# pymc-devs/pymc

Hardware: AMD Instinct MI355X
Metric: effective samples/sec (and leapfrog steps/sec), 10k-param hierarchical logistic regression, one NUTS chain per GPU (higher is better)
Workload: dtype f64

## Files before the change

pymc_amd/csrc/engine.hip:

```cpp
#include <hip/hip_runtime.h>

#include <algorithm>
#include <atomic>
#include <chrono>
#include <cmath>
#include <cstdio>
#include <cstdlib>
#include <cstring>
#include <mutex>
#include <thread>
#include <utility>
#include <ctime>
#include <string>
#include <vector>

#include "kernels.h"
#include "small_kernel.h"
#include "mixture_kernel.h"
#include "loglik_kernel.h"
#include "predictive_kernel.h"
#include "summary_kernel.h"
#include "nuts_mi355.h"
#include "pcg64_stream.h"
#include "advi.h"
// ... 17 lines not shown
static int env_int(const char* name, int dflt) {
  std::lock_guard<std::mutex> lk(g_opt_mu);
  for (const auto& kv : g_opts) if (kv.first == name) return kv.second;
  return dflt;
}
extern "C" int nuts_set_option(const char* name, int32_t value) {
  if (!name || std::strncmp(name, "NUTS_", 5) != 0) { g_err = "option names start with NUTS_"; return NUTS_E_ARG; }
  std::lock_guard<std::mutex> lk(g_opt_mu);
  for (auto& kv : g_opts) if (kv.first == name) { kv.second = value; return NUTS_OK; }
  g_opts.emplace_back(name, value);
  return NUTS_OK;
}
extern "C" void nuts_clear_options(void) {
  std::lock_guard<std::mutex> lk(g_opt_mu);
  g_opts.clear();
}

template <typename T>
static T* dev_alloc(size_t count) {
  void* p = nullptr;
  const size_t bytes = std::max<size_t>(count, 1) * sizeof(T);
  if (hipMalloc(&p, bytes) != hipSuccess) return nullptr;
  if (env_int("NUTS_POISON_ALLOC", 0)) { hipMemset(p, 0xFF, bytes); hipDeviceSynchronize(); }
  return static_cast<T*>(p);
}
template <typename T>
static T* dev_upload(const T* src, size_t count) {
  T* p = dev_alloc<T>(count);
  if (p && count) hipMemcpy(p, src, count * sizeof(T), hipMemcpyHostToDevice);
  return p;
}

enum { EP_PLAIN = 0, EP_PAIRED = 1, EP_REPLAY = 2 };
struct EdgePlan {
  int ring = 64;
  int side = 0, n = 0;
  unsigned head = 0;
  int cap = 0, used = 0;
  int64_t ring_full = 0;
  void reset() { side = 0; n = 0; cap = 0; used = 0; }
  template <class F>
  void begin(int d, int dir, int last, F dir_of) {
    cap = 0; used = 0;
    for (int e = d + 1; e <= last; ++e)
      if (dir_of(e) == -dir) { cap = std::min(1 << std::min(e, 30), ring); break; }
  }
  int leaf(int dir, int* slot, int* k) {
    if (n > 0 && side == dir) { *slot = (int)(head % (unsigned)ring); *k = used++; ++head; --n; return EP_REPLAY; }
    if (cap > 0 && n < cap) { side = -dir; *k = n; *slot = (int)((head + (unsigned)n) % (unsigned)ring); ++n; return EP_PAIRED; }
    if (cap > 0 && n >= ring) ++ring_full;
    *slot = -1; *k = -1;
    return EP_PLAIN;
  }
};
extern "C" int64_t nuts_edge_pair_plan(const int32_t* dirs, int32_t n_dirs, int32_t n_doublings, int32_t spec, int32_t max_depth,
                                       int32_t ring, int32_t* out, int64_t out_cap) {
  if (!dirs || !out || n_doublings < 0 || n_doublings > n_dirs || n_doublings > 20 || ring < 1) { g_err = "nuts_edge_pair_plan: bad argument"; return -1; }
  EdgePlan ep;
  ep.ring = ring;
  int64_t n = 0;
  const int last = std::min(std::min(spec, max_depth - 1), n_dirs - 1);
  for (int d = 0; d < n_doublings; ++d) {
    ep.begin(d, dirs[d], last, [&](int e) { return (int)dirs[e]; });
    for (int j = 0; j < (1 << d); ++j, ++n) {
      int slot, k;
      const int kind = ep.leaf(dirs[d], &slot, &k);
// ... 17 lines not shown
  double* g_dev = nullptr;
  double* lp_dev = nullptr;
  double* host_pin = nullptr;
  std::vector<nuts_data_ref> data_refs;
  int64_t data_epoch = 0;
  double* set_pin = nullptr; int64_t set_pin_len = 0; hipEvent_t set_ev = nullptr;
  int rows_grid = 0, mvn_grid = 0, ept = 1;
  bool has_prog = false;
  int rows_rpl = 2, rows_alternate = 1, rows_flip = 0, rows_occ = 4;
  int vector_one_xcd = 0;
  int ga_struct_ok = 0;
  int ga_par = 0;
  int64_t dom_units = 0;
  int explicit_pre = 0;
  int64_t alg_bytes = 0;
  bool profile = false;
  std::vector<hipEvent_t> ev;
  std::vector<int32_t> ev_units;
  int run_open = 0;
  int64_t runs_seen = 0;
  size_t ev_used = 0;
  int64_t dom_launches = 0;
  int sample_every = 1;
  hipStream_t own_stream = nullptr;
  struct nuts_group* group = nullptr;
  bool g_active = false;
  int gslot = 0;
  int n_chains = 0;
  int64_t pool_extra = 0;
  int64_t orphan_elems = 0, factor_elems = 0;
  double rows_pack_s = 0.0;
  int64_t rows_xt_len = 0, rows_y_len = 0;
  int ep_ok = 0, ep_par = 0;
  double *ep_ring = nullptr, *ep_part = nullptr, *ep_bpart = nullptr, *ep_def_loc = nullptr;
  int64_t ep_ring_bytes = 0, ep_shadows = 0, ep_replays = 0;
  int64_t ep_dropped = 0;
  int64_t ep_ring_full = 0;
  int ep_turns = 0;
  struct EpLaunch {
    int kind = EP_PLAIN, slot = 0, sj = 0, sfold = 0, first = 0;
    EvalIO sio{}; ArenaDev sA{};
  } ep_launch;
  std::vector<LinDev> lins_host;
  std::vector<nuts_factor> fac_host;
  double *ll_q = nullptr, *ll_stage = nullptr, *ll_par = nullptr, *ll_sc = nullptr, *ll_lfact = nullptr;
  int32_t* ll_dead = nullptr;
  int64_t ll_stage_n = 0, ll_par_n = 0;
  int n_waic = 0;

  template <typename T>
  T* keep(T* p) {
    owned.push_back((void*)p);
    return p;
  }
};

extern "C" int nuts_device_count(void) {
  int n = 0;
  if (hipGetDeviceCount(&n) != hipSuccess) return 0;
  return n;
}
extern "C" int nuts_set_device(int device) {
  HIPCHK(hipSetDevice(device));
  return NUTS_OK;
}
extern "C" const char* nuts_last_error(void) { return g_err.c_str(); }
// ... 351 lines not shown
#undef GLM_LAUNCH
    if (prof) { hipEventRecord(m->ev[m->ev_used + 1], m->stream); m->ev_used += 2; m->dom_units += 1; }
    m->dom_launches++;
    hipLaunchKernelGGL(k_glm_reduce, dim3((md.glm.Ppad + 3 + GLM_RED_COLS - 1) / GLM_RED_COLS), dim3(GLM_RED_CHUNKS * GLM_RED_COLS), 0, m->stream, md, A, io, j);
    if (!md.has_mvn) return;
    prof = false; m->dom_launches--;
  }
  if (md.has_logit && md.lg.ga) {
    const int rev = m->rows_alternate ? (m->rows_flip ^= 1) : 0;
    const int par = (m->ga_par ^= 1);
    const dim3 grid(m->rows_grid + (fold ? 1 : 0) + md.lg.ga_naux), block(WAVE * md.lg.ga_w);
    GaArgs ga{md, A, io, j, rev, fold ? (GA_FOLD_CTL | GA_FOLD_SRC) : 0, par, d, max_depth, Emax, st, io, j - 1, d, 0, 0};
    if (fold && job) {
      ga.fold = GA_FOLD_CTL | (job->src_prev ? GA_FOLD_SRC : 0);
      ga.cio = job->io; ga.cj = job->j; ga.cd = job->d; ga.cseq = job->seq;
    }
    const nuts_model::EpLaunch ep = m->ep_launch;
    m->ep_launch.kind = EP_PLAIN;
    if (ep.kind == EP_PAIRED) {
      GaMultiArgs<2, true> ma;
      GaLeafArgs& L = ma.c[0];
      L.A = A; L.io = io; L.cio = ga.cio; L.Emax = Emax; L.st = st;
      L.ga_part = md.lg.ga_part; L.ga_bpart = md.lg.ga_bpart; L.ga_ticket = md.lg.ga_ticket; L.def_loc = md.def_loc;
      L.j = j; L.fold = ga.fold; L.par = par; L.d = d; L.max_depth = max_depth; L.cj = ga.cj; L.cd = ga.cd; L.cseq = ga.cseq;
      L.slot = 0; L.pad = 0;
      GaLeafArgs& S = ma.c[1];
      S.A = ep.sA; S.io = ep.sio; S.cio = ep.sio; S.Emax = Emax; S.st = nullptr;
      S.ga_part = m->ep_part; S.ga_bpart = m->ep_bpart; S.ga_ticket = md.lg.ga_ticket + md.lg.ga_nblk; S.def_loc = m->ep_def_loc;
      S.j = ep.sj; S.fold = ep.sfold; S.par = (m->ep_par ^= 1); S.d = 0; S.max_depth = 1; S.cj = 0; S.cd = 0; S.cseq = 0;
      S.slot = GAM_MAXC - 1; S.pad = ep.first ? GAM_SH_FIRST : 0;
      ma.rev = rev; ma.pad = 0;
      ma.ring = m->ep_ring + (size_t)ep.slot * md.lg.G * GA_RING_DOUBLES(8);
      const dim3 pgrid(GAM_MAXC + md.lg.G);
      if (md.lg.ga_dx == 7) hipLaunchKernelGGL((k_rows_ga_multi<2, 3, 7, true>), pgrid, block, 0, m->stream, md, ma);
      else hipLaunchKernelGGL((k_rows_ga_multi<2, 3, 8, true>), pgrid, block, 0, m->stream, md, ma);
      m->ep_shadows++;
    } else if (ep.kind == EP_REPLAY) {
      const dim3 rgrid(m->rows_grid + (fold ? 1 : 0));
      hipLaunchKernelGGL((k_rows_ga_replay<8>), rgrid, block, 0, m->stream, ga,
                         (const double*)(m->ep_ring + (size_t)ep.slot * md.lg.G * GA_RING_DOUBLES(8)));
      m->ep_replays++;
    } else
    if (m->group && m->g_active && io.mode == MODE_TREE && m->group->kind >= 2) {
      GaLeafArgs L;
      L.A = A; L.io = io; L.cio = ga.cio; L.Emax = Emax; L.st = st;
      L.ga_part = md.lg.ga_part; L.ga_bpart = md.lg.ga_bpart; L.ga_ticket = md.lg.ga_ticket; L.def_loc = md.def_loc;
      L.j = j; L.fold = ga.fold; L.par = par; L.d = d; L.max_depth = max_depth; L.cj = ga.cj; L.cd = ga.cd; L.cseq = ga.cseq;
      L.slot = m->gslot; L.pad = 0;
      group_deposit(m, L);
    } else
    if (md.lg.ga_gpw) {
      switch (md.lg.D) {
        case 8: if (md.lg.ga_dx == 7) hipLaunchKernelGGL((k_rows_gb<8, 7>), grid, block, 0, m->stream, ga);
                else hipLaunchKernelGGL((k_rows_gb<8>), grid, block, 0, m->stream, ga); break;
        case 4: hipLaunchKernelGGL((k_rows_gb<4>), grid, block, 0, m->stream, ga); break;
        case 2: hipLaunchKernelGGL((k_rows_gb<2>), grid, block, 0, m->stream, ga); break;
        case 1: hipLaunchKernelGGL((k_rows_gb<1>), grid, block, 0, m->stream, ga); break;
        case 3: hipLaunchKernelGGL((k_rows_gb<3>), grid, block, 0, m->stream, ga); break;
        case 5: hipLaunchKernelGGL((k_rows_gb<5>), grid, block, 0, m->stream, ga); break;
        case 6: hipLaunchKernelGGL((k_rows_gb<6>), grid, block, 0, m->stream, ga); break;
        default: hipLaunchKernelGGL((k_rows_gb<7>), grid, block, 0, m->stream, ga); break;
      }
    } else {
      switch (md.lg.D) {
        case 8: if (md.lg.ga_pack) hipLaunchKernelGGL((k_rows_ga<8, 2, 7, 1>), grid, block, 0, m->stream, ga);
                else if (md.lg.ga_dx == 7) hipLaunchKernelGGL((k_rows_ga<8, 2, 7>), grid, block, 0, m->stream, ga);
                else hipLaunchKernelGGL((k_rows_ga<8, 2>), grid, block, 0, m->stream, ga); break;
        case 4: hipLaunchKernelGGL((k_rows_ga<4, 2>), grid, block, 0, m->stream, ga); break;
// ... 657 lines not shown
        int t = -1;
        for (int u = 0; u < md.n_derived; ++u) if (md.derived_f[u] == fi) t = u;
        if (t < 0) { g_err = "linear predictor: coefficients must be a variable or a NUTS_D_DERIVED factor"; return false; }
        const int64_t sz = cs.fac[fi].size;
        if (last >= sz) { g_err = "linear predictor: coefficients beyond the end of their derived vector"; return false; }
        C.transform = -1; C.lower = 0.0; C.upper = 0.0;
        cbase = md.derived_off[t]; dst_base = const_cast<double*>(md.pool) + md.derived_off[t] + sz;
      }
      for (int p = 0; p < L.P; ++p) {
        const int64_t e = (int64_t)L.off[k] + (int64_t)p * L.stride[k];
        coef[(size_t)k * L.P + p] = (int32_t)(cbase + e);
        if (C.n_use > 0) srcs.push_back(Src{(int64_t)reinterpret_cast<intptr_t>(dst_base + e), LinSrc{l, k, p, 0}, dst_base + e});
      }
    }
    D.coef = m->keep(dev_upload(coef.data(), coef.size()));
    m->alg_bytes += 16 * L.N * (int64_t)L.P;
  }
  std::stable_sort(srcs.begin(), srcs.end(), [](const Src& a, const Src& b) { return a.key < b.key; });
  std::vector<LinTarget> targets;
  std::vector<LinSrc> flat;
  for (size_t i = 0; i < srcs.size(); ++i) {
    if (i == 0 || srcs[i].key != srcs[i - 1].key) targets.push_back(LinTarget{srcs[i].dst, (int32_t)flat.size(), 0});
    targets.back().n_src++;
    flat.push_back(srcs[i].src);
  }
  md.n_lins = s->n_lins; md.n_lin_targets = (int32_t)targets.size();
  md.lins = m->keep(dev_upload(m->lins_host.data(), m->lins_host.size()));
  md.lin_targets = m->keep(dev_upload(targets.data(), targets.size()));
  md.lin_srcs = m->keep(dev_upload(flat.data(), flat.size()));
  return true;
}

static bool build_rows_group(nuts_model* m, const nuts_model_spec* s, const std::vector<int64_t>& gptr, const std::vector<int32_t>& tile0,
                             int64_t maxT, int W, int gpw) {
  RowsDev& lg = m->md.lg;
  const int n = m->md.n, D = lg.D, SPAN = WAVE * m->rows_rpl;
  const int64_t n_tiles = tile0[lg.G];
  lg.ga = 1; lg.ga_w = gpw ? GB_W : W;
  lg.ga_gpw = gpw;
  lg.ga_bsz = gpw ? gpw : (lg.G + 31) / 32;
  lg.ga_flags = env_int("NUTS_GA_FLAGS", 0);
  lg.ga_T_uni = 0; lg.ga_ng_uni = 0;
  {
    bool uni = lg.G > 0;
    for (int g = 1; g < lg.G; ++g) uni = uni && (gptr[g + 1] - gptr[g] == gptr[1] - gptr[0]);
    if (uni && maxT > 0) { lg.ga_T_uni = (int32_t)maxT; lg.ga_ng_uni = gptr[1] - gptr[0]; }
  }
  lg.ga_nblk = (lg.G + lg.ga_bsz - 1) / lg.ga_bsz;
  lg.ga_auxel = n - lg.G * D;
  lg.ga_naux = m->ga_struct_ok == 2 ? (lg.ga_auxel + WAVE * lg.ga_w - 1) / (WAVE * lg.ga_w) : 0;
  lg.ga_nrec = lg.ga_nblk + lg.ga_naux;
  bool ones0 = D == 8 && env_int("NUTS_GA_ONES0", 1) != 0 && lg.N > 0;
  for (int64_t i = 0; ones0 && i < lg.N; ++i) ones0 = s->rows_X[i * D] == 1.0;
  const int DX = ones0 ? D - 1 : D;
  lg.ga_dx = DX;
  const int64_t TS = (int64_t)DX * SPAN, GA_SKEW = env_int("NUTS_GA_SKEW", DX == 7 || DX == 5 ? 1120 : 1056);
  if (GA_SKEW % DX != 0) return refuse("NUTS_GA_SKEW must be a multiple of the stored column count");
  std::vector<int64_t> coff((size_t)lg.G * W, 0);
  int64_t pos = 0, max_ct = 0;
  for (int g = 0; g < lg.G; ++g) {
    const int64_t T = tile0[g + 1] - tile0[g];
    for (int w = 0; w < W; ++w) {
      const int64_t ct = (int64_t)(w + 1) * T / W - (int64_t)w * T / W;
      coff[(size_t)g * W + w] = pos;
      pos += ct * TS + GA_SKEW;
      max_ct = std::max(max_ct, ct);
    }
// ... 62 lines not shown
      }
      exc.push_back(RpExc{0, 0, 0, 0});
      lg.Xp = m->keep(dev_upload(xp.data(), xp.size()));
      lg.ga_pcoff = m->keep(dev_upload(pcoff.data(), pcoff.size()));
      lg.ga_pexc_idx = m->keep(dev_upload(exc_idx.data(), exc_idx.size()));
      lg.ga_pexc = m->keep(dev_upload(exc.data(), exc.size()));
      lg.ga_pack_ebase20 = (uint32_t)plan.elo << 20;
      lg.ga_pack = (lg.Xp && lg.ga_pcoff && lg.ga_pexc_idx && lg.ga_pexc) ? 1 : 0;
      if (!lg.ga_pack) (void)hipGetLastError();
    }
    m->rows_pack_s = std::chrono::duration<double>(std::chrono::steady_clock::now() - t0).count();
  }
  lg.ga_coff = m->keep(dev_upload(coff.data(), coff.size()));
  lg.ga_tile0 = m->keep(dev_upload(tile0.data(), tile0.size()));
  lg.ga_part = m->keep(dev_alloc<double>((size_t)lg.G * PART_STRIDE));
  const size_t bpart_len = gpw ? 2 * (size_t)PART_STRIDE * ((lg.ga_nrec + WAVE - 1) / WAVE * WAVE) : 2 * (size_t)lg.ga_nrec * PART_STRIDE;
  lg.ga_bpart = m->keep(dev_alloc<double>(bpart_len));
  lg.ga_ticket = m->keep(dev_alloc<unsigned>(2 * (size_t)lg.ga_nblk));
  if (lg.ga_part) hipMemset(lg.ga_part, 0, (size_t)lg.G * PART_STRIDE * sizeof(double));
  if (lg.ga_bpart) hipMemset(lg.ga_bpart, 0, bpart_len * sizeof(double));
  if (lg.ga_ticket) hipMemset(lg.ga_ticket, 0, 2 * (size_t)lg.ga_nblk * sizeof(unsigned));
  m->ep_ok = 0;
  if (!gpw && D == 8 && m->rows_rpl == 2 && m->ga_struct_ok == 1 && lg.ga_naux == 0 && env_int("NUTS_EDGE_PAIR", 1) != 0) {
    const size_t ring_len = (size_t)GA_RING_LEAVES * lg.G * GA_RING_DOUBLES(8);
    m->ep_ring = m->keep(dev_alloc<double>(ring_len));
    m->ep_part = m->keep(dev_alloc<double>((size_t)lg.G * PART_STRIDE));
    m->ep_bpart = m->keep(dev_alloc<double>(bpart_len));
    m->ep_def_loc = m->keep(dev_alloc<double>(2 * 4 * (size_t)MAX_DEFERRED));
    if (m->ep_ring && m->ep_part && m->ep_bpart && m->ep_def_loc) {
      hipMemset(m->ep_part, 0, (size_t)lg.G * PART_STRIDE * sizeof(double));
      hipMemset(m->ep_bpart, 0, bpart_len * sizeof(double));
      hipMemset(m->ep_def_loc, 0, 2 * 4 * (size_t)MAX_DEFERRED * sizeof(double));
      m->ep_ok = 1; m->ep_ring_bytes = (int64_t)(ring_len * sizeof(double));
    } else (void)hipGetLastError();
  }
  m->rows_grid = gpw ? lg.ga_nblk : lg.G;
  return true;
}

static bool build_rows_spans(nuts_model* m, const nuts_model_spec* s, int cus) {
  RowsDev& lg = m->md.lg;
  const int D = lg.D, SPAN = WAVE * m->rows_rpl;
  const int32_t* gid = s->rows_gid;
  int wpc = env_int("NUTS_ROWS_WAVES_PER_CU", 0);
  if (wpc <= 0) {
    const int64_t spans = (s->rows_N + (int64_t)WAVE * m->rows_rpl - 1) / ((int64_t)WAVE * m->rows_rpl);
    wpc = spans >= (int64_t)cus * 32 * 4 ? 32 : 16;
  }
  {
    std::vector<double> xt((size_t)D * lg.Npad, 0.0);
    for (int64_t i = 0; i < lg.N; ++i) {
      const int64_t sp = i / SPAN, r = i % SPAN;
      for (int d = 0; d < D; ++d) xt[((size_t)sp * D + d) * SPAN + r] = s->rows_X[i * D + d];
    }
    lg.Xt = m->keep(dev_upload(xt.data(), xt.size()));
  }
  std::vector<int8_t> yy(lg.Npad, 0);
  for (int64_t i = 0; i < lg.N; ++i) yy[i] = s->rows_y[i];
  lg.y = m->keep(dev_upload(yy.data(), yy.size()));
  const int waves_per_block = ROWS_BLOCK / WAVE;
  int64_t want_waves = std::min<int64_t>((int64_t)cus * wpc, lg.n_spans);
  const int nb_main = (int)((want_waves + waves_per_block - 1) / waves_per_block);
  lg.n_waves = nb_main * waves_per_block;
  std::vector<int32_t> span_gid(lg.n_spans), mixed_g0, mixed_seg_base, mixed_seg_gid;
  std::vector<int64_t> mixed_span;
  for (int64_t sp = 0; sp < lg.n_spans; ++sp) {
// ... 86 lines not shown
    if (i > 0 && gid[i] < gid[i - 1]) return refuse("logit rows: group ids must be sorted");
    if (gid[i] < 0 || gid[i] >= lg.G) return refuse("logit rows: group id out of range");
    gptr[gid[i] + 1] = i + 1;
  }
  for (int g = 0; g < lg.G; ++g) gptr[g + 1] = std::max(gptr[g + 1], gptr[g]);
  lg.gptr = m->keep(dev_upload(gptr.data(), gptr.size()));
  const int want = (s->rows_opts & NUTS_ROWS_NO_GROUP_ALIGNED) ? 0 : env_int("NUTS_ROWS_GA", 1);
  std::vector<int32_t> tile0(lg.G + 1, 0);
  int64_t maxT = 0;
  for (int g = 0; g < lg.G; ++g) {
    const int64_t T = (gptr[g + 1] - gptr[g] + SPAN - 1) / SPAN;
    maxT = std::max(maxT, T);
    tile0[g + 1] = tile0[g] + (int32_t)T;
  }
  const int64_t n_tiles = tile0[lg.G];
  int W = std::min(GA_MAXW, (16 * cus) / std::max(lg.G, 1));
  if (env_int("NUTS_ROWS_GA_W", 0) > 0) W = std::max(1, std::min(GA_MAXW, env_int("NUTS_ROWS_GA_W", 0)));
  const double meanT = (double)n_tiles / std::max(lg.G, 1);
  bool use = false;
  if (want >= 2) { use = m->ga_struct_ok && m->ept == 1; W = std::max(1, W); }
  else if (want == 1) use = m->ga_struct_ok && m->ept == 1 && W >= 1 && lg.G >= 2 * cus && meanT >= 4.0 * W && (double)maxT <= 1.5 * meanT + 1.0;
  int gpw = 0;
  if (!use && want == 1 && !(s->rows_opts & NUTS_ROWS_NO_GROUP_BLOCK) && env_int("NUTS_ROWS_GB", 1) && m->ga_struct_ok && m->ept == 1 &&
      lg.G >= 64 && maxT <= 16) {
    gpw = GB_W * (int)((lg.G + GB_W * 512 - 1) / (GB_W * 512));
    gpw = std::min(gpw, GB_MAXGPW);
    if (env_int("NUTS_ROWS_GPW", 0) > 0) gpw = std::max(1, std::min(GB_MAXGPW, env_int("NUTS_ROWS_GPW", 0)));
    const int aux_threads = WAVE * GB_W, auxel = n - lg.G * D;
    const int naux = m->ga_struct_ok == 2 ? (auxel + aux_threads - 1) / aux_threads : 0;
    if ((lg.G + gpw - 1) / gpw + naux > WAVE * SLOT_SUM_MAXR) gpw = 0;
  }
  if (gpw) { use = true; W = 1; }
  const bool group = use && n_tiles * (int64_t)SPAN < ((int64_t)1 << 31) && (gpw || lg.G <= 32 * 8 * GA_MAXCHUNK);
  if (!(group ? build_rows_group(m, s, gptr, tile0, maxT, W, gpw) : build_rows_spans(m, s, cus))) return false;
  m->alg_bytes += lg.N * (8 * (int64_t)D + 1 + 4);
  return true;
}

static bool build_mvn(nuts_model* m, const nuts_model_spec* s) {
  ModelDev& md = m->md;
  if (s->mvn_k <= 0) return true;
  const int n = md.n;
  md.has_mvn = 1;
  m->explicit_pre = 1;
  MvnDev& mv = md.mv;
  mv.k = s->mvn_k; mv.off = s->vars[s->mvn_var].offset;
  mv.mu = m->keep(dev_upload(s->mvn_mu, mv.k));
  mv.prec = m->keep(dev_upload(s->mvn_prec, (size_t)mv.k * mv.k));
  mv.rowq = m->keep(dev_alloc<double>(mv.k));
  mv.gdense = m->keep(dev_alloc<double>(n));
  hipMemset(mv.gdense, 0, n * sizeof(double));
  mv.konst = -0.5 * mv.k * std::log(2.0 * M_PI) - s->mvn_logdet;
  mv.winv = nullptr; mv.winv_t = nullptr; mv.wy = nullptr;
  if (s->mvn_winv) {
    const size_t kk = (size_t)mv.k * mv.k;
    std::vector<double> wt(kk);
    for (int r = 0; r < mv.k; ++r)
      for (int cc = 0; cc < mv.k; ++cc) wt[(size_t)cc * mv.k + r] = s->mvn_winv[(size_t)r * mv.k + cc];
    mv.winv = m->keep(dev_upload(s->mvn_winv, kk));
    mv.winv_t = m->keep(dev_upload(wt.data(), kk));
    mv.wy = m->keep(dev_alloc<double>(3 * (size_t)mv.k));
  }
  m->mvn_grid = mv.k;
  m->alg_bytes += 8 * (int64_t)mv.k * mv.k;
  mv.aligned = 0; mv.al_nwg = 0; mv.al_part = nullptr;
  if (md.lean_ok && !md.has_logit && !mv.winv && mv.off == 0 && mv.k == n && s->n_vars == 1 && s->n_factors == 0 &&
      s->vars[0].transform == NUTS_TR_NONE && md.n_deferred == 0 && md.n_orphans == 0) {
// ... 161 lines not shown
  md.has_glm = 1;
  m->alg_bytes += 8 * gm.N * (int64_t)gm.P;
  return true;
}

static bool model_build(nuts_model* m, const nuts_model_spec* s) {
  ModelDev& md = m->md;
  HIPCHK_FALSE(hipStreamCreateWithFlags(&m->stream, hipStreamNonBlocking));
  m->own_stream = m->stream;
  int n = 0;
  for (int i = 0; i < s->n_vars; ++i) n = std::max(n, s->vars[i].offset + s->vars[i].size);
  md.n = n; md.n_vars = s->n_vars; md.n_factors = s->n_factors; md.n_data = s->n_data;
  md.fdead_mode = 0;
  md.fdead = m->keep(dev_alloc<int32_t>((size_t)std::max(s->n_factors, 1)));
  if (md.fdead) hipMemset(md.fdead, 0, (size_t)std::max(s->n_factors, 1) * sizeof(int32_t));
  CompiledSpec cs;
  if (!compile_spec(m, s, cs)) return false;
  m->fac_host = cs.fac;
  {
    double* pool = m->keep(dev_alloc<double>((size_t)std::max<int64_t>(s->data_pool_len + m->pool_extra, 1)));
    if (pool) {
      hipMemset(pool, 0, (size_t)std::max<int64_t>(s->data_pool_len + m->pool_extra, 1) * sizeof(double));
      if (s->data_pool_len > 0) hipMemcpy(pool, s->data_pool, (size_t)s->data_pool_len * sizeof(double), hipMemcpyHostToDevice);
    }
    md.pool = pool;
    md.pool_len = (int32_t)std::min<int64_t>(s->data_pool_len + m->pool_extra, INT32_MAX);
  }
  m->data_refs.assign(s->data, s->data + s->n_data);
  m->ept = n <= 65536 ? 1 : (n <= 262144 ? 4 : 16);
  md.nblk = (n + VEC_THREADS * m->ept - 1) / (VEC_THREADS * m->ept);
  if (m->orphan_elems > 4 * VEC_THREADS * (int64_t)md.nblk)
    md.nblk = (int)std::min<int64_t>(256, (m->orphan_elems + 4 * VEC_THREADS - 1) / (4 * VEC_THREADS));
  md.tick_j = env_int("NUTS_TICK_J", -1);
  md.ticks = m->keep(dev_alloc<long long>(64));
  hipMemset(md.ticks, 0, 64 * sizeof(long long));
  md.part_stride = PART_STRIDE;
  m->vector_one_xcd = env_int("NUTS_VECTOR_ONE_XCD", 0);
  md.part = m->keep(dev_alloc<double>((size_t)md.nblk * PART_STRIDE));
  hipMemset(md.part, 0, (size_t)md.nblk * PART_STRIDE * sizeof(double));
  m->q_dev = m->keep(dev_alloc<double>(n));
  m->g_dev = m->keep(dev_alloc<double>(n));
  m->lp_dev = m->keep(dev_alloc<double>(2));
  HIPCHK_FALSE(hipHostMalloc((void**)&m->host_pin, (2 * (size_t)n + 2) * sizeof(double), hipHostMallocDefault));
  m->alg_bytes = 0;

  hipDeviceProp_t prop;
  int dev = 0;
  hipGetDevice(&dev);
  hipGetDeviceProperties(&prop, dev);
  const int cus = prop.multiProcessorCount > 0 ? prop.multiProcessorCount : 256;
  if (!build_rows(m, s, cus) || !build_mvn(m, s) || !build_mix(m, s, cs) || !build_glm(m, s, cs, cus) || !build_lins(m, s, cs) ||
      !build_sweep_fast(m, s, cs))
    return false;
  for (void* p : m->owned)
    if (!p) return refuse("device allocation failed");
  HIPCHK_FALSE(hipDeviceSynchronize());
  return true;
}

extern "C" nuts_model* nuts_model_create(const nuts_model_spec* s) {
  if (!s || s->n_vars <= 0) { g_err = "empty model spec"; return nullptr; }
  int ndev = 0;
  if (hipGetDeviceCount(&ndev) != hipSuccess || ndev == 0) {
    g_err = "no HIP device visible: libnuts_mi355 requires an MI355X (gfx950); there is no CPU fallback";
    return nullptr;
  }
  auto* m = new nuts_model();
  if (!model_build(m, s)) { nuts_model_destroy(m); return nullptr; }
// ... 35 lines not shown
    const int64_t off0 = m->data_refs[data_ids[i]].offset;
    int64_t run = lens[i];
    int j = i + 1;
    while (j < count && m->data_refs[data_ids[j]].offset == off0 + run) { run += lens[j]; ++j; }
    if (run > 0)
      HIPCHK(hipMemcpyAsync(const_cast<double*>(m->md.pool) + off0, m->set_pin + at, (size_t)run * sizeof(double), hipMemcpyHostToDevice, m->stream));
    at += run;
    i = j;
  }
  HIPCHK(hipEventRecord(m->set_ev, m->stream));
  m->data_epoch++;
  return NUTS_OK;
}

static void group_remove_model(struct nuts_group* g, nuts_model* m);
extern "C" void nuts_model_destroy(nuts_model* m) {
  if (!m) return;
  if (m->stream) hipStreamSynchronize(m->stream);
  if (m->set_ev) hipEventDestroy(m->set_ev);
  if (m->set_pin) hipHostFree(m->set_pin);
  if (m->group) group_remove_model(m->group, m);
  for (void* p : m->owned) if (p) hipFree(p);
  for (void* p : {(void*)m->ll_q, (void*)m->ll_stage, (void*)m->ll_par, (void*)m->ll_sc, (void*)m->ll_dead, (void*)m->ll_lfact}) if (p) hipFree(p);
  for (auto e : m->ev) hipEventDestroy(e);
  if (m->host_pin) hipHostFree(m->host_pin);
  if (m->own_stream) hipStreamDestroy(m->own_stream);
  delete m;
}

extern "C" int nuts_model_debug_ticks(nuts_model* m, int64_t* out) {
  if (!m || !out) return NUTS_E_ARG;
  HIPCHK(hipStreamSynchronize(m->stream));
  HIPCHK(hipMemcpy(out, m->md.ticks, 64 * sizeof(long long), hipMemcpyDeviceToHost));
  return NUTS_OK;
}

extern "C" int32_t nuts_model_ndim(const nuts_model* m) { return m ? m->md.n : -1; }
extern "C" int nuts_model_get_scalar(const nuts_model* m, const char* name, double* out) {
  if (!m || !name || !out) return NUTS_E_ARG;
  const std::string k(name);
  if (k == "rows_group_aligned") *out = m->md.lg.ga;
  else if (k == "rows_group_block") *out = m->md.lg.ga_gpw;
  else if (k == "rows_packed") *out = m->md.lg.ga ? m->md.lg.ga_pack : 0;
  else if (k == "rows_pack_build_s") *out = m->rows_pack_s;
  else if (k == "edge_pair") *out = m->ep_ok;
  else if (k == "edge_pair_ring_bytes") *out = (double)m->ep_ring_bytes;
  else if (k == "edge_pair_shadows") *out = (double)m->ep_shadows;
  else if (k == "edge_pair_replays") *out = (double)m->ep_replays;
  else if (k == "edge_pair_turns") *out = m->ep_turns;
  else if (k == "edge_pair_dropped") *out = (double)m->ep_dropped;
  else if (k == "edge_pair_ring_full") *out = (double)m->ep_ring_full;
  else if (k == "rows_aux_workgroups") *out = m->md.lg.ga ? m->md.lg.ga_naux : 0;
  else if (k == "mixture_workgroups") *out = m->md.has_mix ? m->md.mix.nwg : 0;
  else if (k == "glm_workgroups") *out = m->md.has_glm ? m->md.glm.nwg : 0;
  else if (k == "glm_row_stride") *out = m->md.has_glm ? m->md.glm.xstride : 0;
  else if (k == "glm_layout_width") *out = m->md.has_glm ? m->md.glm.Ppad : 0;
  else if (k == "mvn_row_aligned") *out = m->md.has_mvn ? m->md.mv.aligned : 0;
  else if (k == "loglik_batch") *out = LL_B;
  else if (k == "loglik_stage_bytes") *out = (double)(m->ll_stage_n * LL_B * (int64_t)sizeof(double));
  else if (k == "rows_waves") *out = m->md.lg.ga ? m->md.lg.ga_w : m->md.lg.n_waves;
  else if (k == "lean") *out = m->md.lean_ok;
  else if (k == "chain_group_kind") {
    const RowsDev& lg = m->md.lg;
    const bool is_mvn = m->md.has_mvn && (m->md.mv.aligned == 4 || m->md.mv.aligned == 8 || m->md.mv.aligned == 16);
    const bool is_rows = m->md.has_logit && !m->md.has_mvn && lg.ga && lg.ga_naux == 0 && lg.D == 8 && m->ga_struct_ok == 1;
    *out = is_mvn ? 1.0 : (is_rows ? (lg.ga_gpw > 0 ? 3.0 : 2.0) : 0.0);
  }
  else if (k == "chain_group_wide_ok") *out = (m->md.has_mvn && m->md.mv.aligned > 0 && m->md.mv.k % 16 == 0) ? 1.0 : 0.0;
  else if (k == "chain_group_wide_rows") *out = 8.0;
  else if (k == "single_workgroup_ok") *out = (m->md.n <= SMALL_MAX_N && m->ept == 1 && !m->md.has_logit && !m->md.has_mvn && !m->md.has_mix && !m->md.has_glm && m->md.n_lins == 0 && m->factor_elems <= SMALL_MAX_ELEMS) ? 1.0 : 0.0;
  else { g_err = "unknown model scalar " + k; return NUTS_E_ARG; }
  return NUTS_OK;
}
extern "C" int64_t nuts_model_algorithmic_bytes(const nuts_model* m) { return m ? m->alg_bytes : 0; }

extern "C" int nuts_model_logp_grad(nuts_model* m, const double* q, double* logp, double* grad) {
  if (!m || !q || !logp) { g_err = "null argument"; return NUTS_E_ARG; }
  const int n = m->md.n;
  std::memcpy(m->host_pin, q, n * sizeof(double));
  HIPCHK(hipMemcpyAsync(m->q_dev, m->host_pin, n * sizeof(double), hipMemcpyHostToDevice, m->stream));
  m->md.fdead_mode = 1;
  model_enqueue_plain(m, m->q_dev, m->g_dev, m->lp_dev);
  m->md.fdead_mode = 0;
  HIPCHK(hipMemcpyAsync(m->host_pin + n, m->g_dev, n * sizeof(double), hipMemcpyDeviceToHost, m->stream));
// ... 2754 lines not shown
```

pymc_amd/csrc/model_dev.h:

```cpp
#pragma once
#include "device_math.h"
#include "nuts_mi355.h"
#include "rows_pack.h"

#define MAX_BTERMS 8
#define MAX_DERIVED 4
#define MAX_FACTOR_BT 6
#define MAX_DEFERRED 256
#define LOGIT_MAXD 8
#define SEG_MAIN_MAX 10

struct VarDev {
  int32_t offset, size, transform, deferred;
  double lower, upper;
  int32_t normal_prior;
  int32_t def_base;
  double np_mu, np_inv_var, np_lognorm;
};

struct Contrib {
  int32_t f;
  int16_t arg, slot;
  int32_t owner;
  int32_t fast;
// ... 173 lines not shown
  int64_t derived_off[MAX_DERIVED];
  const char* prog;
  int32_t po_vars, po_cptr, po_contrib, po_factors, po_fbt, po_btvar, po_data, po_deferred, po_instrs, po_pad;
  long long* ticks;
  int32_t tick_j;
  int32_t fdead_mode;
  int32_t* fdead;
  int32_t n_gsf, n_gs_elems;
  int32_t po_gsf, po_gslot;
  int32_t n_gs_blocks, n_orphans_b;
  double* gs_part;
  int32_t n_swf, sw_bytes, sw_rows, sw_po_leaf, sw_po_instr, sw_po_slot;
  int32_t sw_max_leaves, sw_max_slots, sw_max_instr, sw_blocks;
  const char* sw_blob;
  int32_t gs_lds_rows, gs_lds_bytes;
  double* adj;
  int32_t n_glong, glong_pad;
  const GLong* glong;
  double* adj_red;
  int32_t n_lins, n_lin_targets;
  const LinDev* lins;
  const LinTarget* lin_targets;
  const LinSrc* lin_srcs;
  double* lin_gdense;
};

#ifdef NUTS_KTIMING
__device__ __forceinline__ long long tick_now() {
  unsigned long long t;
  asm volatile("s_waitcnt vmcnt(0) lgkmcnt(0)\n\ts_memtime %0\n\ts_waitcnt lgkmcnt(0)" : "=s"(t) :: "memory");
  return (long long)t;
}
#define TICK(md, cond, slot) do { if (cond) (md).ticks[slot] = tick_now(); } while (0)
#else
#define TICK(md, cond, slot) do { } while (0)
#endif

__device__ __forceinline__ void st_agent(double* p, double v) {
  __hip_atomic_store(reinterpret_cast<unsigned long long*>(p), (unsigned long long)__double_as_longlong(v), __ATOMIC_RELAXED,
                     __HIP_MEMORY_SCOPE_AGENT);
}
__device__ __forceinline__ double ld_agent(const double* p) {
  return __longlong_as_double((long long)__hip_atomic_load(reinterpret_cast<const unsigned long long*>(p), __ATOMIC_RELAXED,
                                                           __HIP_MEMORY_SCOPE_AGENT));
}

template <int BATCH = 8>
__device__ __forceinline__ double sum_strided(const double* base, int stride, int s0, int s1) {
  double acc = 0.0;
  for (int s = s0; s < s1; s += BATCH) {
    double v[BATCH];
#pragma unroll
    for (int u = 0; u < BATCH; ++u) v[u] = base[(int64_t)min(s + u, s1 - 1) * stride];
#pragma unroll
    for (int u = 0; u < BATCH; ++u) acc += (s + u < s1) ? v[u] : 0.0;
  }
  return acc;
}

#define CTL_CHUNKS 8

__device__ __forceinline__ double deferred_finish(double gx_local, double S, double dxdq, double dj) {
  return fma(gx_local + S, dxdq, dj);
}

#define PROG_LDS_MAX 12288

// ... 783 lines not shown
```

pymc_amd/csrc/rows_ga_multi_kernel.h:

```cpp
#pragma once
#include "mvn_multi_kernel.h"

#define GAM_MAXC 8
#define GAM_MAXNC 4

struct GaLeafArgs {
  ArenaDev A;
  EvalIO io, cio;
  double Emax;
  HostStatus* st;
  double* ga_part;
  double* ga_bpart;
  unsigned* ga_ticket;
  double* def_loc;
  int j, fold, par, d, max_depth, cj, cd, cseq;
  int slot, pad;
};

template <int NC, bool SH = false>
struct GaMultiArgs {
  GaLeafArgs c[NC];
  int rev, pad;
};
#define GAM_SH_FIRST 1
template <int NC>
struct GaMultiArgs<NC, true> {
  GaLeafArgs c[NC];
  int rev, pad;
  double* ring;
};

__device__ __forceinline__ LeanSrc gam_src(const RowsDev& R, const GaLeafArgs& L, int par) {
  return LeanSrc{L.ga_bpart + (int64_t)par * R.ga_nrec * PART_STRIDE, PART_STRIDE, R.ga_nrec, L.def_loc + (int64_t)par * 4 * MAX_DEFERRED};
}

template <int DX>
__device__ __forceinline__ void gam_load(const double* base , const int8_t* ybase, int lane,
                                         typename GaTileSel<DX>::type& t) {
  const ga_v2d* p = reinterpret_cast<const ga_v2d*>(base) + lane;
#pragma unroll
  for (int k = 0; k < DX; ++k) t.c[k] = p[k * WAVE];
  t.y = *reinterpret_cast<const uint16_t*>(ybase + 2 * lane);
}

template <int NC, int OCC, int DX, bool SH = false>
__global__ __launch_bounds__(64 * GA_MAXW, OCC) void k_rows_ga_multi(ModelDev md, GaMultiArgs<NC, SH> ma) {
  constexpr int D = 8, RPL = 2, SPAN = WAVE * RPL, PIPE = 2;
  static_assert(!SH || NC == 2, "edge pairing: the chain's leaf and one shadow leaf");
  typedef GaMultiArgs<NC, SH> Args;
  typedef typename GaTileSel<DX>::type Tile;
  const RowsDev& R = md.lg;
  if ((int)blockIdx.x < GAM_MAXC) {
    int ci = -1;
#pragma unroll
    for (int c = 0; c < NC; ++c) ci = (int)blockIdx.x == ma.c[c].slot ? c : ci;
    if (ci < 0) return;
    const GaLeafArgs& L = ma.c[ci];
    if (L.fold & GA_FOLD_CTL) control_lean(md, L.A, L.cio, L.cj, L.cd, L.Emax, L.max_depth, L.st, L.cseq, gam_src(R, L, L.par ^ 1));
    return;
  }
  const int g = (int)blockIdx.x - GAM_MAXC;
  const int rev = ma.rev;
  const int tid = threadIdx.x, lane = tid & (WAVE - 1), w = __builtin_amdgcn_readfirstlane(tid >> 6), W = (int)blockDim.x >> 6;
  __shared__ double s_acc[NC][GA_MAXW][2][D + 1];
  __shared__ double s_red[NC][NDOT];
  __shared__ double s_cp[GA_MAXCHUNK][PART_STRIDE];
  __shared__ int s_info[NC][4];
  __shared__ double s_keep[NC][5][WAVE];
  __shared__ double s_beta[NC][D];
  __shared__ __attribute__((aligned(16))) char s_args[(sizeof(Args) + 15) / 16 * 16];

  int T; int64_t ng, cbase;
  if (R.ga_T_uni > 0) { T = R.ga_T_uni; ng = R.ga_ng_uni; cbase = (int64_t)(g * W + w) * R.ga_cstride_uni; }
  else {
    T = __builtin_amdgcn_readfirstlane(R.ga_tile0[g + 1] - R.ga_tile0[g]);
    ng = __builtin_amdgcn_readfirstlane((int)(R.gptr[g + 1] - R.gptr[g]));
    const int64_t cb = R.ga_coff[g * W + w];
    cbase = ((int64_t)__builtin_amdgcn_readfirstlane((int)(cb >> 32)) << 32) | (uint32_t)__builtin_amdgcn_readfirstlane((int)(cb & 0xffffffffll));
  }
  const int c0 = (int)((int64_t)w * T / W), c2 = (int)((int64_t)(w + 1) * T / W);
  const int n = c2 - c0;
  const int nA = (n + 1) / 2;
  const int nsw = rev ? n - nA : nA;
  constexpr int64_t TS = (int64_t)DX * SPAN;
  auto local_at = [&](int i) { return rev ? (i < nsw ? nA + i : i - nsw) : i; };
  auto tile_at = [&](int i) { return cbase + (int64_t)local_at(i) * TS; };
  const int l_last = (c2 == T) ? n - 1 : -1;
  const int n_last = (int)(ng - (int64_t)(T - 1) * SPAN);
  if (lane == 0) {
#pragma unroll
    for (int c = 0; c < NC; ++c)
#pragma unroll
      for (int dd = 0; dd <= D; ++dd) { s_acc[c][w][0][dd] = 0.0; s_acc[c][w][1][dd] = 0.0; }
  }
  {
    static_assert(alignof(Args) == 8 && sizeof(Args) % 8 == 0, "kernarg layout: the second argument follows the model at the next multiple of 8");
    const uint2* ka = (const uint2*)__builtin_amdgcn_kernarg_segment_ptr() + (sizeof(ModelDev) + 7) / 8;
    for (int t = tid; t < (int)(sizeof(Args) / 8); t += (int)blockDim.x) reinterpret_cast<uint2*>(s_args)[t] = ka[t];
  }

  int dead = 0;
#pragma unroll
  for (int c = 0; c < NC; ++c) dead |= load_aborted(ma.c[c].io, ma.c[c].A) ? (1 << c) : 0;
  if constexpr (SH) dead = (dead & 1) ? 3 : 0;
  if (dead == (1 << NC) - 1) return;
  for (int c = w; c < NC; c += W) {
    const GaLeafArgs& L = ma.c[c];
    Leaf lf; QView qv;
    double hval0, hph0;
    if (SH && c == 1 && (L.pad & GAM_SH_FIRST)) {
      resolve_leaf(L.io, ma.c[0].A, L.j, lf, qv);
      ga_hyper<D>(R, qv, L.fold, gam_src(R, ma.c[0], ma.c[0].par ^ 1), lane, hval0, hph0);
    } else {
      resolve_leaf(L.io, L.A, L.j, lf, qv);
      ga_hyper<D>(R, qv, L.fold, gam_src(R, L, L.par ^ 1), lane, hval0, hph0);
    }
    const int dl = lane % D;
    const int iz = R.off_z + g * D + dl;
    double zq, zph, m_lane, s_lane;
    ga_z_state(qv, iz, zq, zph);
    ga_hyper_lanes<D>(R, hval0, dl, m_lane, s_lane);
    const double bl = fma(s_lane, zq, m_lane);
    if (lane < D) s_beta[c][lane] = bl;
    s_keep[c][0][lane] = hval0; s_keep[c][1][lane] = hph0; s_keep[c][2][lane] = zq; s_keep[c][3][lane] = zph; s_keep[c][4][lane] = s_lane;
  }
  __syncthreads();
  constexpr bool TWO = NC <= 3;
  Tile ta, tb;
  {
    const int64_t o0 = tile_at(0), o1 = tile_at(min(1, max(n - 1, 0)));
    gam_load<DX>(R.Xt + o0, R.y + o0 / DX, lane, ta);
    if constexpr (TWO) gam_load<DX>(R.Xt + o1, R.y + o1 / DX, lane, tb);
  }
  double beta[NC][D];
#pragma unroll
  for (int c = 0; c < NC; ++c)
#pragma unroll
    for (int dd = 0; dd < D; ++dd) beta[c][dd] = readlane_d(s_beta[c][dd], 0);

  {
    double acc[NC][D], lp[NC];
#pragma unroll
    for (int c = 0; c < NC; ++c) {
      lp[c] = 0.0;
#pragma unroll
      for (int dd = 0; dd < D; ++dd) acc[c][dd] = 0.0;
    }
    int half = rev ? 1 : 0;
    auto flush = [&]() {
      double flat[NC * D];
#pragma unroll
      for (int c = 0; c < NC; ++c)
#pragma unroll
        for (int dd = 0; dd < D; ++dd) flat[c * D + dd] = acc[c][dd];
      int idx;
      const double t = wave_sum_many<NC * D>(flat, lane, idx);
      constexpr int NVP = NC * D <= 8 ? 8 : NC * D <= 16 ? 16 : 32;
      if (lane < NVP && idx < NC * D) s_acc[idx / D][w][half][idx % D] = t;
      int idx2;
      const double t2 = wave_sum_many<NC>(lp, lane, idx2);
      constexpr int NVP2 = NC <= 1 ? 1 : NC <= 2 ? 2 : 4;
      if (lane < NVP2 && idx2 < NC) s_acc[idx2][w][half][D] = t2;
#pragma unroll
      for (int c = 0; c < NC; ++c) {
        lp[c] = 0.0;
#pragma unroll
        for (int dd = 0; dd < D; ++dd) acc[c][dd] = 0.0;
      }
      half ^= 1;
    };
    const int nm1 = n - 1;
    auto issue = [&](int i, Tile& t) {
      const int64_t off = tile_at(min(i, nm1));
      gam_load<DX>(R.Xt + off, R.y + off / DX, lane, t);
    };
#define GAM_STAGE(TT, I)                                                                     \
    {                                                                                        \
      if ((I) == nsw) flush();                                                               \
      double xx[8][2];                                                                       \
      ga_unpack(TT, xx);                                                                     \
      const uint32_t yy = TT.y;                                                              \
      const int nv = local_at(I) == l_last ? n_last : SPAN;                                  \
       \
      _Pragma("unroll") for (int c = 0; c < NC; ++c) ga_tile<8, 2, (NC == 2)>(xx, yy, beta[c], nv, lane, acc[c], lp[c]); \
    }
    if constexpr (TWO) {
      for (int i = 0; i < n; i += 2) {
        GAM_STAGE(ta, i)
        if (i + 1 >= n) break;
        issue(i + 2, ta);
        GAM_STAGE(tb, i + 1)
        issue(i + 3, tb);
      }
    } else {
      for (int i = 0; i < n; ++i) {
        GAM_STAGE(ta, i)
        issue(i + 1, ta);
      }
    }
#undef GAM_STAGE
    if (n > 0) flush();
  }

  const Args& Tm = *reinterpret_cast<const Args*>(s_args);
  MergePrefetch mpf;
  if (w < NC && !((dead >> w) & 1) && !(SH && w == 1)) {
    const GaLeafArgs& L = Tm.c[w];
    Leaf lf; QView qv;
    resolve_leaf(L.io, L.A, L.j, lf, qv);
    merge_prefetch(L.A, lf, L.j, R.off_z + g * D + lane % D, mpf);
  }
  __syncthreads();
  if constexpr (SH) {
    constexpr int NR = GA_RING_DOUBLES(D);
    for (int t = tid; t < NR; t += (int)blockDim.x) Tm.ring[(int64_t)g * NR + t] = (&s_acc[1][0][0][0])[t];
  }
  for (int c = w; c < NC; c += W) {
    if ((dead >> c) & 1) { if (lane == 0) s_info[c][0] = 0; continue; }
    const GaLeafArgs& L = Tm.c[c];
    Leaf lf; QView qv;
    resolve_leaf(L.io, L.A, L.j, lf, qv);
    if (SH && c == 1) {
      ga_tail_wave<D, false>(R, L.A, L.io, L.ga_part, L.ga_ticket, L.def_loc, lf, g, W, L.j, L.par, L.d, s_acc[c], s_red[c], s_info[c],
                             s_keep[c][0][lane], s_keep[c][1][lane], s_keep[c][2][lane], s_keep[c][3][lane], s_keep[c][4][lane], nullptr);
      continue;
    }
    auto tail = [&](const MergePrefetch* pf) {
      ga_tail_wave<D, true>(R, L.A, L.io, L.ga_part, L.ga_ticket, L.def_loc, lf, g, W, L.j, L.par, L.d, s_acc[c], s_red[c], s_info[c],
                            s_keep[c][0][lane], s_keep[c][1][lane], s_keep[c][2][lane], s_keep[c][3][lane], s_keep[c][4][lane], pf);
    };
    if (c == w) tail(&mpf);
    else tail(nullptr);
  }
  __syncthreads();
#pragma unroll
  for (int c = 0; c < NC; ++c) {
    if (!s_info[c][0]) continue;
    ga_block_partial<D>(R, Tm.c[c].ga_part, Tm.c[c].ga_bpart, Tm.c[c].par, g, true, s_info[c], s_cp);
    __syncthreads();
  }
}
```

Measured before the change: 20250.

## Raise edge-pairing kernel occupancy, add packed-tile path and single-buffer pipeline

The paired-leaf rows kernel now launches with four waves per SIMD instead of three, so the whole grid is meant to stay resident. It gains a packed-tile variant that reads compressed tiles and patches exception entries, plus a single-buffered load loop that lowers register pressure. Host code picks the variant from the packing state and computes residency rounds through the occupancy API. Per-workgroup timing ticks are added under a debug macro. The risk is extra unpack and patch work, and less latency hiding with only one prefetched tile.

```diff
diff --git a/pymc_amd/csrc/engine.hip b/pymc_amd/csrc/engine.hip
--- a/pymc_amd/csrc/engine.hip
+++ b/pymc_amd/csrc/engine.hip
@@ -73,6 +73,7 @@
 }
 
 enum { EP_PLAIN = 0, EP_PAIRED = 1, EP_REPLAY = 2 };
+enum { EPV_PACKED = 0, EPV_RAW7 = 1, EPV_RAW8 = 2 };
 struct EdgePlan {
   int ring = 64;
   int side = 0, n = 0;
@@ -156,6 +157,8 @@
   double rows_pack_s = 0.0;
   int64_t rows_xt_len = 0, rows_y_len = 0;
   int ep_ok = 0, ep_par = 0;
+  int ep_variant = 0;
+  int ep_rounds = 0;
   double *ep_ring = nullptr, *ep_part = nullptr, *ep_bpart = nullptr, *ep_def_loc = nullptr;
   int64_t ep_ring_bytes = 0, ep_shadows = 0, ep_replays = 0;
   int64_t ep_dropped = 0;
@@ -573,8 +576,11 @@
       ma.rev = rev; ma.pad = 0;
       ma.ring = m->ep_ring + (size_t)ep.slot * md.lg.G * GA_RING_DOUBLES(8);
       const dim3 pgrid(GAM_MAXC + md.lg.G);
-      if (md.lg.ga_dx == 7) hipLaunchKernelGGL((k_rows_ga_multi<2, 3, 7, true>), pgrid, block, 0, m->stream, md, ma);
-      else hipLaunchKernelGGL((k_rows_ga_multi<2, 3, 8, true>), pgrid, block, 0, m->stream, md, ma);
+      switch (m->ep_variant) {
+        case EPV_PACKED: hipLaunchKernelGGL((k_rows_ga_multi<2, 4, 7, true, 1>), pgrid, block, 0, m->stream, md, ma); break;
+        case EPV_RAW7: hipLaunchKernelGGL((k_rows_ga_multi<2, 4, 7, true>), pgrid, block, 0, m->stream, md, ma); break;
+        default: hipLaunchKernelGGL((k_rows_ga_multi<2, 4, 8, true>), pgrid, block, 0, m->stream, md, ma); break;
+      }
       m->ep_shadows++;
     } else if (ep.kind == EP_REPLAY) {
       const dim3 rgrid(m->rows_grid + (fold ? 1 : 0));
@@ -1298,7 +1304,7 @@
 }
 
 static bool build_rows_group(nuts_model* m, const nuts_model_spec* s, const std::vector<int64_t>& gptr, const std::vector<int32_t>& tile0,
-                             int64_t maxT, int W, int gpw) {
+                             int64_t maxT, int W, int gpw, int cus) {
   RowsDev& lg = m->md.lg;
   const int n = m->md.n, D = lg.D, SPAN = WAVE * m->rows_rpl;
   const int64_t n_tiles = tile0[lg.G];
@@ -1427,6 +1433,17 @@
       hipMemset(m->ep_bpart, 0, bpart_len * sizeof(double));
       hipMemset(m->ep_def_loc, 0, 2 * 4 * (size_t)MAX_DEFERRED * sizeof(double));
       m->ep_ok = 1; m->ep_ring_bytes = (int64_t)(ring_len * sizeof(double));
+      m->ep_variant = lg.ga_pack ? EPV_PACKED : (DX == 7 ? EPV_RAW7 : EPV_RAW8);
+      const void* kfn = nullptr;
+      switch (m->ep_variant) {
+        case EPV_PACKED: kfn = (const void*)k_rows_ga_multi<2, 4, 7, true, 1>; break;
+        case EPV_RAW7: kfn = (const void*)k_rows_ga_multi<2, 4, 7, true>; break;
+        default: kfn = (const void*)k_rows_ga_multi<2, 4, 8, true>; break;
+      }
+      int per_cu = 0;
+      if (hipOccupancyMaxActiveBlocksPerMultiprocessor(&per_cu, kfn, WAVE * W, 0) != hipSuccess || per_cu < 1) { (void)hipGetLastError(); per_cu = 0; }
+      const int64_t slots = (int64_t)per_cu * cus, wgs = (int64_t)GAM_MAXC + lg.G;
+      m->ep_rounds = slots > 0 ? (int)((wgs + slots - 1) / slots) : 0;
     } else (void)hipGetLastError();
   }
   m->rows_grid = gpw ? lg.ga_nblk : lg.G;
@@ -1579,7 +1596,7 @@
   }
   if (gpw) { use = true; W = 1; }
   const bool group = use && n_tiles * (int64_t)SPAN < ((int64_t)1 << 31) && (gpw || lg.G <= 32 * 8 * GA_MAXCHUNK);
-  if (!(group ? build_rows_group(m, s, gptr, tile0, maxT, W, gpw) : build_rows_spans(m, s, cus))) return false;
+  if (!(group ? build_rows_group(m, s, gptr, tile0, maxT, W, gpw, cus) : build_rows_spans(m, s, cus))) return false;
   m->alg_bytes += lg.N * (8 * (int64_t)D + 1 + 4);
   return true;
 }
@@ -1807,8 +1824,8 @@
   if (m->orphan_elems > 4 * VEC_THREADS * (int64_t)md.nblk)
     md.nblk = (int)std::min<int64_t>(256, (m->orphan_elems + 4 * VEC_THREADS - 1) / (4 * VEC_THREADS));
   md.tick_j = env_int("NUTS_TICK_J", -1);
-  md.ticks = m->keep(dev_alloc<long long>(64));
-  hipMemset(md.ticks, 0, 64 * sizeof(long long));
+  md.ticks = m->keep(dev_alloc<long long>(TICK_SLOTS));
+  hipMemset(md.ticks, 0, TICK_SLOTS * sizeof(long long));
   md.part_stride = PART_STRIDE;
   m->vector_one_xcd = env_int("NUTS_VECTOR_ONE_XCD", 0);
   md.part = m->keep(dev_alloc<double>((size_t)md.nblk * PART_STRIDE));
@@ -1910,6 +1927,27 @@
   if (!m || !out) return NUTS_E_ARG;
   HIPCHK(hipStreamSynchronize(m->stream));
   HIPCHK(hipMemcpy(out, m->md.ticks, 64 * sizeof(long long), hipMemcpyDeviceToHost));
+#ifdef NUTS_KTIMING
+  if (m->md.has_logit && m->md.lg.ga && m->ep_ok) {
+    const int nw = std::min(m->md.lg.G, EP_TICK_WG);
+    std::vector<long long> wg(2 * (size_t)nw);
+    HIPCHK(hipMemcpy(wg.data(), m->md.ticks + 64, wg.size() * sizeof(long long), hipMemcpyDeviceToHost));
+    long long n = 0, s0 = 0, e0 = 0, e1 = 0, s1 = 0;
+    for (int g = 0; g < nw; ++g) {
+      const long long a = wg[2 * (size_t)g], b = wg[2 * (size_t)g + 1];
+      if (a == 0 || b < a) continue;
+      s0 = n ? std::min(s0, a) : a; e0 = n ? std::min(e0, b) : b; e1 = n ? std::max(e1, b) : b; s1 = n ? std::max(s1, a) : a;
+      ++n;
+    }
+    long long late = 0, late_max = 0, late_sum = 0;
+    for (int g = 0; g < nw; ++g) {
+      const long long a = wg[2 * (size_t)g], b = wg[2 * (size_t)g + 1];
+      if (a == 0 || b < a || a <= e0) continue;
+      ++late; late_max = std::max(late_max, a); late_sum += a - e0;
+    }
+    out[40] = n; out[41] = s0; out[42] = e0; out[43] = e1; out[44] = late; out[45] = late_max; out[46] = late_sum; out[47] = s1;
+  }
+#endif
   return NUTS_OK;
 }
 
@@ -1928,6 +1966,8 @@
   else if (k == "edge_pair_turns") *out = m->ep_turns;
   else if (k == "edge_pair_dropped") *out = (double)m->ep_dropped;
   else if (k == "edge_pair_ring_full") *out = (double)m->ep_ring_full;
+  else if (k == "edge_pair_packed") *out = m->ep_ok && m->ep_variant == EPV_PACKED ? 1.0 : 0.0;
+  else if (k == "edge_pair_rounds") *out = m->ep_ok ? m->ep_rounds : 0;
   else if (k == "rows_aux_workgroups") *out = m->md.lg.ga ? m->md.lg.ga_naux : 0;
   else if (k == "mixture_workgroups") *out = m->md.has_mix ? m->md.mix.nwg : 0;
   else if (k == "glm_workgroups") *out = m->md.has_glm ? m->md.glm.nwg : 0;
diff --git a/pymc_amd/csrc/model_dev.h b/pymc_amd/csrc/model_dev.h
--- a/pymc_amd/csrc/model_dev.h
+++ b/pymc_amd/csrc/model_dev.h
@@ -229,7 +229,15 @@
   return (long long)t;
 }
 #define TICK(md, cond, slot) do { if (cond) (md).ticks[slot] = tick_now(); } while (0)
+__device__ __forceinline__ long long tick_real() {
+  unsigned long long t;
+  asm volatile("s_waitcnt vmcnt(0) lgkmcnt(0)\n\ts_memrealtime %0\n\ts_waitcnt lgkmcnt(0)" : "=s"(t) :: "memory");
+  return (long long)t;
+}
+#define EP_TICK_WG 4096
+#define TICK_SLOTS (64 + 2 * EP_TICK_WG)
 #else
+#define TICK_SLOTS 64
 #define TICK(md, cond, slot) do { } while (0)
 #endif
 
diff --git a/pymc_amd/csrc/rows_ga_multi_kernel.h b/pymc_amd/csrc/rows_ga_multi_kernel.h
--- a/pymc_amd/csrc/rows_ga_multi_kernel.h
+++ b/pymc_amd/csrc/rows_ga_multi_kernel.h
@@ -43,12 +43,22 @@
   t.y = *reinterpret_cast<const uint16_t*>(ybase + 2 * lane);
 }
 
-template <int NC, int OCC, int DX, bool SH = false>
+__device__ __forceinline__ void gam_load_packed(const uint32_t* base , int lane, GaTileRegsP& t) {
+  const ga_v4u* p = reinterpret_cast<const ga_v4u*>(base) + lane;
+#pragma unroll
+  for (int k = 0; k < 6; ++k) t.p[k] = p[k * WAVE];
+  t.last = base[6 * 4 * WAVE + lane];
+}
+
+template <int NC, int OCC, int DX, bool SH = false, int PK = 0>
 __global__ __launch_bounds__(64 * GA_MAXW, OCC) void k_rows_ga_multi(ModelDev md, GaMultiArgs<NC, SH> ma) {
   constexpr int D = 8, RPL = 2, SPAN = WAVE * RPL, PIPE = 2;
   static_assert(!SH || NC == 2, "edge pairing: the chain's leaf and one shadow leaf");
+  static_assert(!SH || OCC == 4, "edge pairing: four waves per SIMD, the whole grid resident");
+  static_assert(!PK || (SH && DX == 7), "packed tiles: the edge-pairing launch of a model with seven stored columns");
+  constexpr bool ONE = SH;
   typedef GaMultiArgs<NC, SH> Args;
-  typedef typename GaTileSel<DX>::type Tile;
+  typedef typename GaTileSel<DX, PK>::type Tile;
   const RowsDev& R = md.lg;
   if ((int)blockIdx.x < GAM_MAXC) {
     int ci = -1;
@@ -60,6 +70,9 @@
     return;
   }
   const int g = (int)blockIdx.x - GAM_MAXC;
+#ifdef NUTS_KTIMING
+  const long long tk_top = tick_real();
+#endif
   const int rev = ma.rev;
   const int tid = threadIdx.x, lane = tid & (WAVE - 1), w = __builtin_amdgcn_readfirstlane(tid >> 6), W = (int)blockDim.x >> 6;
   __shared__ double s_acc[NC][GA_MAXW][2][D + 1];
@@ -71,18 +84,20 @@
   __shared__ __attribute__((aligned(16))) char s_args[(sizeof(Args) + 15) / 16 * 16];
 
   int T; int64_t ng, cbase;
-  if (R.ga_T_uni > 0) { T = R.ga_T_uni; ng = R.ga_ng_uni; cbase = (int64_t)(g * W + w) * R.ga_cstride_uni; }
+  int tg0;
+  if (R.ga_T_uni > 0) { T = R.ga_T_uni; ng = R.ga_ng_uni; cbase = (int64_t)(g * W + w) * (PK ? R.ga_pstride_uni : R.ga_cstride_uni); tg0 = g * T; }
   else {
-    T = __builtin_amdgcn_readfirstlane(R.ga_tile0[g + 1] - R.ga_tile0[g]);
+    tg0 = __builtin_amdgcn_readfirstlane(R.ga_tile0[g]);
+    T = __builtin_amdgcn_readfirstlane(R.ga_tile0[g + 1]) - tg0;
     ng = __builtin_amdgcn_readfirstlane((int)(R.gptr[g + 1] - R.gptr[g]));
-    const int64_t cb = R.ga_coff[g * W + w];
+    const int64_t cb = (PK ? R.ga_pcoff : R.ga_coff)[g * W + w];
     cbase = ((int64_t)__builtin_amdgcn_readfirstlane((int)(cb >> 32)) << 32) | (uint32_t)__builtin_amdgcn_readfirstlane((int)(cb & 0xffffffffll));
   }
   const int c0 = (int)((int64_t)w * T / W), c2 = (int)((int64_t)(w + 1) * T / W);
   const int n = c2 - c0;
   const int nA = (n + 1) / 2;
   const int nsw = rev ? n - nA : nA;
-  constexpr int64_t TS = (int64_t)DX * SPAN;
+  constexpr int64_t TS = PK ? RP_TILE_DWORDS : (int64_t)DX * SPAN;
   auto local_at = [&](int i) { return rev ? (i < nsw ? nA + i : i - nsw) : i; };
   auto tile_at = [&](int i) { return cbase + (int64_t)local_at(i) * TS; };
   const int l_last = (c2 == T) ? n - 1 : -1;
@@ -125,9 +140,14 @@
     s_keep[c][0][lane] = hval0; s_keep[c][1][lane] = hph0; s_keep[c][2][lane] = zq; s_keep[c][3][lane] = zph; s_keep[c][4][lane] = s_lane;
   }
   __syncthreads();
-  constexpr bool TWO = NC <= 3;
+  constexpr bool TWO = NC <= 3 && !ONE;
   Tile ta, tb;
-  {
+  uint64_t ea = 0;
+  const int te0 = tg0 + c0;
+  if constexpr (PK) {
+    gam_load_packed(R.Xp + tile_at(0), lane, ta);
+    ea = ga_exc_range(R.ga_pexc_idx, te0 + local_at(0));
+  } else {
     const int64_t o0 = tile_at(0), o1 = tile_at(min(1, max(n - 1, 0)));
     gam_load<DX>(R.Xt + o0, R.y + o0 / DX, lane, ta);
     if constexpr (TWO) gam_load<DX>(R.Xt + o1, R.y + o1 / DX, lane, tb);
@@ -171,8 +191,14 @@
     };
     const int nm1 = n - 1;
     auto issue = [&](int i, Tile& t) {
-      const int64_t off = tile_at(min(i, nm1));
-      gam_load<DX>(R.Xt + off, R.y + off / DX, lane, t);
+      const int ii = min(i, nm1);
+      if constexpr (PK) {
+        gam_load_packed(R.Xp + tile_at(ii), lane, t);
+        ea = ga_exc_range(R.ga_pexc_idx, te0 + local_at(ii));
+      } else {
+        const int64_t off = tile_at(ii);
+        gam_load<DX>(R.Xt + off, R.y + off / DX, lane, t);
+      }
     };
 #define GAM_STAGE(TT, I)                                                                     \
     {                                                                                        \
@@ -184,7 +210,25 @@
        \
       _Pragma("unroll") for (int c = 0; c < NC; ++c) ga_tile<8, 2, (NC == 2)>(xx, yy, beta[c], nv, lane, acc[c], lp[c]); \
     }
-    if constexpr (TWO) {
+    if constexpr (ONE) {
+      uint32_t ebase20 = 0;
+      if constexpr (PK) ebase20 = R.ga_pack_ebase20;
+      for (int i = 0; i < n; ++i) {
+        if (i == nsw) flush();
+        double xx[8][2];
+        if constexpr (PK) {
+          ga_unpack(ta, ebase20, xx);
+          if ((uint32_t)(ea >> 32) != 0) ga_patch(R.ga_pexc, ea, lane, xx);
+        } else {
+          ga_unpack(ta, xx);
+        }
+        const uint32_t yy = ga_ybits(ta);
+        const int nv = local_at(i) == l_last ? n_last : SPAN;
+        issue(i + 1, ta);
+#pragma unroll
+        for (int c = 0; c < NC; ++c) ga_tile<8, 2>(xx, yy, beta[c], nv, lane, acc[c], lp[c]);
+      }
+    } else if constexpr (TWO) {
       for (int i = 0; i < n; i += 2) {
         GAM_STAGE(ta, i)
         if (i + 1 >= n) break;
@@ -239,4 +283,10 @@
     ga_block_partial<D>(R, Tm.c[c].ga_part, Tm.c[c].ga_bpart, Tm.c[c].par, g, true, s_info[c], s_cp);
     __syncthreads();
   }
-}
+#ifdef NUTS_KTIMING
+  if constexpr (SH) {
+    __syncthreads();
+    if (tid == 0 && g < EP_TICK_WG) { md.ticks[64 + 2 * g] = tk_top; md.ticks[64 + 2 * g + 1] = tick_real(); }
+  }
+#endif
+}
```

Result: faster. 20740 (median of 6 runs) (+2.4%).
